# pythtb/pythtb

Hardware: AMD Instinct MI355X
Metric: k-points solved/sec (H(k)+eigh) and Berry-flux/sec, Haldane 2048^2 mesh (higher is better)
Workload: dtype f64

## Files before the change

pythtb_amd/csrc/tbk_berry.hip:

```cpp
#include <math.h>
#include <stdlib.h>
#include <string.h>
#include <algorithm>
#include "tbk_internal.h"

struct AxisSet {
    int n;
    int size[3];
    int64_t stride[3];
};

__device__ __forceinline__ int64_t axis_offset(const AxisSet& ax, int64_t s) {
    int64_t off = 0;
#pragma unroll
    for (int a = 2; a >= 0; --a) {
        if (a < ax.n) {
            const int64_t q = s / ax.size[a];
            off += (s - q * ax.size[a]) * ax.stride[a];
            s = q;
        }
    }
    return off;
}

// ... 557 lines not shown
__global__ __launch_bounds__(256) void k_flux(const FluxArgs A) {
    const int slice = blockIdx.x / A.bps;
    const int blk = blockIdx.x - slice * A.bps;
    const unsigned p = (unsigned)blk * 256u + threadIdx.x;
    const unsigned per = (unsigned)A.n0 * (unsigned)A.n1;
    double pha = 0.0;
    if (p < per) {
        const unsigned i = p / (unsigned)A.n1, j = p - i * (unsigned)A.n1;
        const int nc = A.v.ncomp;
        const int64_t plane = A.v.npts * nc;
        const int64_t base = axis_offset(A.other, slice) + (int64_t)i * A.s0 + (int64_t)j * A.s1;
        const cd* u00 = A.v.data + base * nc;
        const cd* u10 = u00 + A.s0 * nc;
        const cd* u01 = u00 + A.s1 * nc;
        const cd* u11 = u10 + A.s1 * nc;
        cd d = one_link_det<NOCC, MAXN>(u00, u10, A.occ, A.nocc, nc, plane);
        d = cmul(d, one_link_det<NOCC, MAXN>(u10, u11, A.occ, A.nocc, nc, plane));
        d = cmul(d, one_link_det<NOCC, MAXN>(u11, u01, A.occ, A.nocc, nc, plane));
        d = cmul(d, one_link_det<NOCC, MAXN>(u01, u00, A.occ, A.nocc, nc, plane));
        pha = -atan2(d.y, d.x);
        if (A.plaq) A.plaq[(int64_t)slice * per + p] = pha;
    }
    __shared__ double red[4];
    double s = pha;
#pragma unroll
    for (int off = 32; off > 0; off >>= 1) s += __shfl_xor(s, off);
    if ((threadIdx.x & 63) == 0) red[threadIdx.x >> 6] = s;
    __syncthreads();
    if (threadIdx.x == 0) A.partial[(int64_t)slice * A.bps + blk] = (red[0] + red[1]) + (red[2] + red[3]);
}

__global__ __launch_bounds__(1024) void k_flux_reduce(const double* __restrict__ partial, int bps,
                                                      double* __restrict__ totals, const DoneArgs done) {
    const double* p = partial + (int64_t)blockIdx.x * bps;
    double s0 = 0.0, s1 = 0.0, s2 = 0.0, s3 = 0.0;
    for (int i = threadIdx.x; i < bps; i += 4 * 1024) {
        const double v0 = p[i];
        const double v1 = i + 1024 < bps ? p[i + 1024] : 0.0;
        const double v2 = i + 2048 < bps ? p[i + 2048] : 0.0;
        const double v3 = i + 3072 < bps ? p[i + 3072] : 0.0;
        s0 += v0;
        s1 += v1;
        s2 += v2;
        s3 += v3;
    }
    double s = (s0 + s1) + (s2 + s3);
#pragma unroll
    for (int off = 32; off > 0; off >>= 1) s += __shfl_xor(s, off);
    __shared__ double red[16];
    if ((threadIdx.x & 63) == 0) red[threadIdx.x >> 6] = s;
    __syncthreads();
    if (threadIdx.x == 0) {
        double t = red[0];
#pragma unroll
        for (int i = 1; i < 16; ++i) t += red[i];
        red[0] = t;
    }
    if (threadIdx.x == 0) {
        totals[blockIdx.x] = red[0];
        tbk_signal_done(done);
    }
}

static int check_occ(const tbk_wfs* w, const int32_t* occ, int nocc) {
    TBK_REQUIRE(occ && nocc >= 1, TBK_EINVAL, "occ must list at least one state");
    for (int i = 0; i < nocc; ++i)
        TBK_REQUIRE(occ[i] >= 0 && occ[i] < w->view.nsta, TBK_EINVAL, "occ[%d]=%d outside 0..%d", i, occ[i],
                    w->view.nsta - 1);
    return TBK_OK;
}

static int fill_occ(const tbk_wfs* w, const int32_t* occ, int nocc, int* dst) {
    int rc = check_occ(w, occ, nocc);
    if (rc) return rc;
    TBK_REQUIRE(nocc <= TBK_MAX_NOCC, TBK_EUNSUPPORTED, "nocc=%d exceeds this build's limit of %d", nocc, TBK_MAX_NOCC);
    for (int i = 0; i < nocc; ++i) dst[i] = occ[i];
    return TBK_OK;
}

#include "tbk_berry_big.inl"
#include "tbk_berry_lanes.inl"

static int big_scratch(tbk_wfs* w, const int32_t* occ, int nocc, int ndirs, size_t extra, int** occ_dev, cd** dets,
                       void** work, size_t* work_bytes, void** extra_dev) {
    tbk_ctx* ctx = w->ctx;
    auto al = [](size_t x) { return (x + 255) & ~(size_t)255; };
    const size_t ob = al((size_t)nocc * sizeof(int));
    const size_t db = al((size_t)w->view.npts * sizeof(cd));
    const size_t per = (size_t)nocc * nocc * sizeof(cd);
    const bool in_lds = (size_t)nocc * (nocc + 1) * sizeof(cd) <= 96 * 1024;
    const size_t wb = in_lds ? 0 : al(per * (size_t)std::min<int64_t>(w->view.npts, (int64_t)ctx->cus * 4));
    void* base = nullptr;
    int rc = tbk_ctx_scratch(ctx, 256 + ob + ndirs * db + wb + al(extra), &base);
    if (rc) return rc;
// ... 20 lines not shown
        ax->stride[ax->n] = v.stride[d];
        ax->n++;
        *count *= v.mesh[d];
    }
}

template <int NOCC, int MAXN>
static void launch_flux(tbk_ctx* ctx, const FluxArgs& A, int64_t nslices) {
    hipLaunchKernelGGL((k_flux<NOCC, MAXN>), dim3((unsigned)(nslices * A.bps)), dim3(256), 0, ctx->stream, A);
}

static int chain_wave_link_dets(tbk_wfs* w, const int32_t* occ, int nocc, int dir, cd* dets_out);
#define TBK_LANES_DET_LDS_MAX ((size_t)128 * 1024)
#define TBK_LANES_FLUX_LDS_MAX ((size_t)72 * 1024)
static bool lanes_dets_applies(const WfsView& v, int nocc, size_t lds_max);
static int lanes_link_dets(tbk_wfs* w, const int32_t* occ, int nocc, int dir, cd* dets_out);
static bool chain_wave_applies(const WfsView& v, int nocc);

extern "C" int tbk_berry_flux_async(tbk_wfs* w, const int32_t* occ, int nocc, int dir0, int dir1,
                                    int want_plaq) {
    TBK_REQUIRE(w, TBK_EINVAL, "tbk_berry_flux: null wfs");
    const WfsView& v = w->view;
    TBK_REQUIRE(dir0 != dir1, TBK_EINVAL, "Need to specify two different directions for Berry flux calculation.");
    TBK_REQUIRE(dir0 >= 0 && dir1 >= 0 && dir0 < v.dim_arr && dir1 < v.dim_arr, TBK_EINVAL,
                "Direction for Berry flux calculation out of bounds.");
    FluxArgs A{};
    int det_from = 9;
    if (tbk_knobs().det_big_from >= 0) det_from = std::max(2, tbk_knobs().det_big_from);
    const bool big = nocc >= det_from;
    int rc = big ? check_occ(w, occ, nocc) : fill_occ(w, occ, nocc, A.occ);
    if (rc) return rc;
    tbk_ctx* ctx = w->ctx;
    TBK_HIP(hipSetDevice(ctx->device));
    A.v = v;
    A.nocc = nocc;
    A.n0 = v.mesh[dir0] - 1;
    A.n1 = v.mesh[dir1] - 1;
    A.s0 = v.stride[dir0];
    A.s1 = v.stride[dir1];
    int64_t nslices = 1;
    other_axes(v, dir0, dir1, &A.other, &nslices);
    const int64_t per = (int64_t)A.n0 * A.n1;
    TBK_REQUIRE(per < (int64_t)0xffffffffu, TBK_EUNSUPPORTED, "plane of %lld plaquettes is too large", (long long)per);
    const bool rows = !big && v.ncomp <= 4 && nocc <= v.ncomp;
    if (rows) {
        A.swap = A.s0 < A.s1;
        A.na = A.swap ? A.n1 : A.n0;
        A.nb = A.swap ? A.n0 : A.n1;
        A.sa = A.swap ? A.s1 : A.s0;
        A.sb = A.swap ? A.s0 : A.s1;
        A.ncolw = (A.nb + 62) / 63;
        const int64_t want = (int64_t)ctx->cus * 12;
        int64_t ti = ((int64_t)A.na * A.ncolw * nslices + want - 1) / want;
        A.ti = (int)std::max<int64_t>(4, std::min<int64_t>(24, ti));
        if (tbk_knobs().flux_ti >= 0) A.ti = std::max(1, tbk_knobs().flux_ti);
        A.bps = ((A.na + A.ti - 1) / A.ti) * A.ncolw;
    } else {
        A.bps = (int)((per + 255) / 256);
    }
    FluxSliceArgs SL{};
    const int Dm = v.dim_arr;
    const bool slices_k = rows && !want_plaq && Dm >= 3 && dir0 != Dm - 1 && dir1 != Dm - 1 && v.mesh[Dm - 1] >= 16 &&
                          tbk_knobs().flux_slices != 0;
    if (slices_k) {
        SL.nfast = v.mesh[Dm - 1];
        SL.ngrp = (SL.nfast + 63) / 64;
// ... 126 lines not shown
            }
#undef TBK_SLC
        } else if (rows) {
            const dim3 grid((unsigned)(nslices * A.bpb)), blk(256);
#define TBK_ROWS(NO, NC) hipLaunchKernelGGL((k_flux_rows<NO, NC>), grid, blk, 0, ctx->stream, A)
            switch (v.ncomp * 8 + nocc) {
                case 1 * 8 + 1: TBK_ROWS(1, 1); break;
                case 2 * 8 + 1: TBK_ROWS(1, 2); break;
                case 2 * 8 + 2: TBK_ROWS(2, 2); break;
                case 3 * 8 + 1: TBK_ROWS(1, 3); break;
                case 3 * 8 + 2: TBK_ROWS(2, 3); break;
                case 3 * 8 + 3: TBK_ROWS(3, 3); break;
                case 4 * 8 + 1: TBK_ROWS(1, 4); break;
                case 4 * 8 + 2: TBK_ROWS(2, 4); break;
                case 4 * 8 + 3: TBK_ROWS(3, 4); break;
                default: TBK_ROWS(4, 4); break;
            }
#undef TBK_ROWS
        } else {
            switch (nocc) {
                case 1: launch_flux<1, 1>(ctx, A, nslices); break;
                case 2: launch_flux<2, 1>(ctx, A, nslices); break;
                case 3: launch_flux<3, 1>(ctx, A, nslices); break;
                case 4: launch_flux<4, 1>(ctx, A, nslices); break;
                case 5: launch_flux<5, 1>(ctx, A, nslices); break;
                case 6: launch_flux<6, 1>(ctx, A, nslices); break;
                case 7: launch_flux<7, 1>(ctx, A, nslices); break;
                case 8: launch_flux<8, 1>(ctx, A, nslices); break;
                default: launch_flux<0, TBK_MAX_NOCC>(ctx, A, nslices);
            }
        }
        TBK_HIP(hipGetLastError());
    }
    if (!rows || !A.fused || slices_k) {
        ProfScope ps(ctx, "flux_reduce");
        w->flux_done = (w->flux_totals_host && !want_plaq) ? tbk_done_arm(ctx, false) : DoneArgs{nullptr, nullptr, nullptr, 0u};
        hipLaunchKernelGGL(k_flux_reduce, dim3((unsigned)nslices), dim3(1024), 0, ctx->stream,
                           (const double*)w->flux_partial_dev, (rows && !slices_k) ? A.bpb : A.bps, w->flux_totals_dev, w->flux_done);
        TBK_HIP(hipGetLastError());
    } else {
        w->flux_done = DoneArgs{nullptr, nullptr, nullptr, 0u};
    }
    return TBK_OK;
}

extern "C" int tbk_berry_flux_result(tbk_wfs* w, double* totals, double* plaq) {
    TBK_REQUIRE(w && totals, TBK_EINVAL, "tbk_berry_flux_result: null argument");
    TBK_REQUIRE(w->flux_nslices > 0, TBK_EINVAL, "tbk_berry_flux_result: no flux launch pending");
    tbk_ctx* ctx = w->ctx;
    if (plaq) {
        TBK_REQUIRE(w->flux_plaq_n > 0, TBK_EINVAL, "tbk_berry_flux_result: plaquettes were not requested");
        TBK_HIP(hipMemcpyAsync(plaq, w->flux_plaq_dev, w->flux_plaq_n * sizeof(double), hipMemcpyDeviceToHost,
                               ctx->stream));
    }
    if (w->flux_totals_host) {
        const DoneArgs done = plaq ? DoneArgs{nullptr, nullptr, nullptr, 0u} : w->flux_done;
        w->flux_done = DoneArgs{nullptr, nullptr, nullptr, 0u};
        const int rc = tbk_done_wait(ctx, done);
        if (rc) return rc;
        memcpy(totals, w->flux_totals_host, w->flux_nslices * sizeof(double));
        return TBK_OK;
    }
    return tbk_small_d2h(ctx, totals, w->flux_totals_dev, w->flux_nslices * sizeof(double));
}

extern "C" int tbk_berry_flux(tbk_wfs* w, const int32_t* occ, int nocc, int dir0, int dir1, double* totals,
                              double* plaq) {
    int rc = tbk_berry_flux_async(w, occ, nocc, dir0, dir1, plaq != nullptr);
    if (rc) return rc;
    return tbk_berry_flux_result(w, totals, plaq);
}

struct ChainArgs {
    WfsView v;
    int nocc;
    int occ[TBK_MAX_NOCC];
    int nlinks;
    int64_t sdir;
    AxisSet other;
    int64_t nstrings;
    int seg_len, nseg;
    int final_lanes;
// ... 1184 lines not shown
```

pythtb_amd/csrc/tbk_core.hip:

```cpp
#include <stdarg.h>
#include <stdio.h>
#include <stdlib.h>
#include <string.h>
#include <algorithm>
#include <array>
#include <chrono>
#include <map>
#include <new>
#include "tbk_internal.h"
#include <cmath>

static thread_local char g_err[1024] = "";

void tbk_set_error(const char* fmt, ...) {
    va_list ap;
    va_start(ap, fmt);
    vsnprintf(g_err, sizeof(g_err), fmt, ap);
    va_end(ap);
}

extern "C" const char* tbk_last_error(void) { return g_err; }

static TbkKnobs g_knobs;
static bool g_knobs_parsed = false;
// ... 18 lines not shown
    geti("TBK_QL32", k.ql32);
    geti("TBK_QLW_STREAMS", k.qlw_streams);
    geti("TBK_QLW_BISECT", k.qlw_bisect);
    geti("TBK_QLW_REPLAY_REG", k.qlw_replay_reg);
    geti("TBK_QLW_WS_MB", k.qlw_ws_mb);
    getl("TBK_QLW_CAP", k.qlw_cap);
    geti("TBK_QL16_EVONLY", k.ql16_evonly);
    geti("TBK_TW16", k.tw16);
    geti("TBK_E16", k.e16);
    geti("TBK_E16_NS_FULL", k.e16_ns_full);
    geti("TBK_E16_CELLS", k.e16_cells);
    geti("TBK_E16_EVALS", k.e16_evals);
    geti("TBK_TW16_STREAMS", k.tw16_streams);
    if (const char* e = getenv("TBK_TW16_GAPTOL")) k.tw16_gaptol = atof(e);
    geti("TBK_QL16_SPLIT", k.ql16_split);
    getl("TBK_QL16_SPLIT_MIN", k.ql16_split_min);
    getl("TBK_QL16_MIN", k.ql16_min);
    getl("TBK_FEW_MAX", k.few_max);
    geti("TBK_FEW_WARM", k.few_warm);
    geti("TBK_FEW_NT", k.few_nt);
    geti("TBK_WG_NT", k.wg_nt);
    geti("TBK_WAVE_RUN", k.wave_run);
    geti("TBK_GRID_SEG", k.grid_seg);
    geti("TBK_FUSED_ROWS", k.fused_rows);
    geti("TBK_FUSED_SUM", k.fused_sum);
    geti("TBK_FUSED_OCC", k.fused_occ);
    geti("TBK_GRID_OCC", k.grid_occ);
    geti("TBK_SMALL_KPT", k.small_kpt);
    geti("TBK_ZERO_COPY_KB", k.zero_copy_kb);
    geti("TBK_GRID_KERNEL", k.grid_kernel);
    geti("TBK_FLUX_TI", k.flux_ti);
    geti("TBK_FLUX_FUSED", k.flux_fused);
    geti("TBK_FLUX_ORDER", k.flux_order);
    geti("TBK_REG_DIRECT", k.reg_direct);
    geti("TBK_REG_CELLS", k.reg_cells);
    geti("TBK_FLUX_SLICES", k.flux_slices);
    geti("TBK_POLL_DONE", k.poll_done);
    geti("TBK_POS_TILE", k.pos_tile);
    geti("TBK_GRID_IMG", k.grid_img);
    geti("TBK_CHAIN_WAVE", k.chain_wave);
    geti("TBK_CHAIN_TILE", k.chain_tile);
    geti("TBK_CHAIN_PROD", k.chain_prod);
    geti("TBK_MESH_ROWS", k.mesh_rows);
    geti("TBK_TRIGV_FROM", k.trigv_from);
    geti("TBK_CHAIN_WS_MB", k.chain_ws_mb);
    geti("TBK_CHAIN_WAVE_FROM", k.chain_wave_from);
    geti("TBK_DET_BIG_FROM", k.det_big_from);
    geti("TBK_WILSON_BIG_FROM", k.wilson_big_from);
    geti("TBK_WILSON_REG", k.wilson_reg);
    geti("TBK_WILSON_SEG", k.wilson_seg);
    geti("TBK_WILSON_SWZ", k.wilson_swz);
    geti("TBK_WILSON_FORM", k.wilson_form);
    geti("TBK_WILSON_MFMA", k.wilson_mfma);
    getl("TBK_WILSON_BATCH_BYTES", k.wilson_batch_bytes);
    if (const char* e = getenv("TBK_WILSON_ALPHA")) {
        k.wilson_alpha = atof(e);
        k.wilson_alpha_set = true;
    }
    getl("TBK_BIG_BATCH", k.big_batch);
#ifdef TBK_REG_MULTILANE
    geti("TBK_REG_LANES", k.reg_lanes);
#endif
#ifdef TBK_DIAG
    geti("TBK_ABLATE_GRID", k.ablate_grid);
    geti("TBK_ABLATE_FLUX", k.ablate_flux);
#endif
// ... 165 lines not shown
    if (!c->done_host || tbk_knobs().poll_done == 0 || c->prof_period != 0) return d;
    c->done_seq += 1u;
    if (c->done_seq == 0u) c->done_seq = 1u;
    d.word = c->done_dev;
    d.cnt = c->done_cnt_dev;
    d.flags_src = with_flags ? c->flags_dev : nullptr;
    d.seq = c->done_seq;
    return d;
}

int tbk_done_wait(tbk_ctx* c, const DoneArgs& d) {
    if (d.word) {
        const volatile unsigned* w = c->done_host;
        const auto t0 = std::chrono::steady_clock::now();
        for (;;) {
            for (int i = 0; i < 512; ++i) {
                if ((int)(__atomic_load_n(w, __ATOMIC_ACQUIRE) - d.seq) >= 0) return TBK_OK;
                __builtin_ia32_pause();
            }
            if (std::chrono::steady_clock::now() - t0 > std::chrono::milliseconds(1)) break;
        }
    }
    TBK_HIP(hipStreamSynchronize(c->stream));
    return TBK_OK;
}

void tbk_wfs_totals_free(tbk_wfs* w) {
    if (w->flux_totals_host) hipHostFree(w->flux_totals_host);
    else if (w->flux_totals_dev) hipFree(w->flux_totals_dev);
    w->flux_totals_host = nullptr;
    w->flux_totals_dev = nullptr;
}
int tbk_wfs_totals_alloc(tbk_wfs* w, int64_t nslices) {
    tbk_wfs_totals_free(w);
    const size_t bytes = (size_t)std::max<int64_t>(nslices, 1) * sizeof(double);
    if (bytes <= 64 * 1024 && tbk_knobs().zero_copy_kb > 0) {
        void* h = nullptr;
        void* d = nullptr;
        if (hipHostMalloc(&h, bytes, hipHostMallocMapped) == hipSuccess && hipHostGetDevicePointer(&d, h, 0) == hipSuccess) {
            w->flux_totals_host = (double*)h;
            w->flux_totals_dev = (double*)d;
            return TBK_OK;
        }
        (void)hipGetLastError();
        if (h) hipHostFree(h);
    }
    TBK_HIP(hipMalloc((void**)&w->flux_totals_dev, bytes));
    return TBK_OK;
}

int tbk_ctx_scratch(tbk_ctx* c, size_t bytes, void** out) {
    if (bytes > c->scratch_bytes) {
        TBK_HIP(hipStreamSynchronize(c->stream));
        if (c->scratch) TBK_HIP(hipFree(c->scratch));
        c->scratch = nullptr;
        c->scratch_bytes = 0;
        size_t want = std::max(bytes, (size_t)1 << 20);
        hipError_t e = hipMalloc(&c->scratch, want);
        if (e != hipSuccess) {
            tbk_set_error("device scratch of %zu bytes: %s", want, hipGetErrorString(e));
            return TBK_ENOMEM;
        }
        c->scratch_bytes = want;
    }
    *out = c->scratch;
    return TBK_OK;
// ... 783 lines not shown
```

pythtb_amd/csrc/tbk_internal.h:

```cpp
#pragma once
#include <hip/hip_runtime.h>
#include <stdint.h>
#include <string>
#include <vector>
#include "../../include/tbk.h"

void tbk_set_error(const char* fmt, ...);

#define TBK_HIP(call)                                                                   \
    do {                                                                                \
        hipError_t e_ = (call);                                                         \
        if (e_ != hipSuccess) {                                                         \
            tbk_set_error("%s failed: %s (%s:%d)", #call, hipGetErrorString(e_),        \
                          __FILE__, __LINE__);                                          \
            return TBK_EHIP;                                                            \
        }                                                                               \
    } while (0)

#define TBK_REQUIRE(cond, code, ...)                                                    \
    do {                                                                                \
        if (!(cond)) {                                                                  \
            tbk_set_error(__VA_ARGS__);                                                 \
            return (code);                                                              \
        }                                                                               \
// ... 21 lines not shown
    int qlw_nt = -1;
    long long qlw_cap = -1;
    int qlw_ws_mb = -1;
    int ql16_split = 1;
    long long ql16_split_min = -1;
    int tw16_streams = -1;
    int e16 = 1;
    int tw16 = 1;
    int e16_evals = 1;
    int e16_cells = 1;
    int e16_ns_full = 0;
    double tw16_gaptol = 1e-5;
    int ql16_evonly = 1;
    long long few_max = -1;
    int few_warm = 1;
    int few_nt = -1;
    int wg_nt = 1024;
    int wave_run = -1;
    int fused_rows = -1;
    int zero_copy_kb = 1024;
    int small_kpt = -1;
    int grid_occ = -1;
    int fused_occ = -1;
    int fused_sum = 1;
    int grid_seg = -1;
    int grid_kernel = 0;
    int flux_ti = -1;
    int grid_img = 1;
    int pos_tile = 1;
    int poll_done = 1;
    int flux_slices = 1;
    int flux_fused = 0;
    int flux_order = -1;
    int trigv_from = -1;
    int chain_ws_mb = 1024;
    int mesh_rows = 1;
    int chain_prod = 1;
    int chain_tile = 1;
    int chain_wave = 1;
    int chain_wave_from = -1;
    int det_big_from = -1;
    int wilson_mfma = 1;
    int wilson_reg = 3;
    int wilson_seg = -1;
    int wilson_swz = 1;
    int wilson_form = -1;
    int wilson_big_from = -1;
    long long wilson_batch_bytes = -1;
    double wilson_alpha = 0.0;
    bool wilson_alpha_set = false;
    long long big_batch = -1;
    int reg_lanes = 0;
    int reg_cells = 1;
    int reg_direct = 1;
    int ablate_grid = 0;
    int ablate_flux = 0;
};
const TbkKnobs& tbk_knobs();

#ifdef TBK_DIAG
#define TBK_ABLATE(expr) (expr)
#else
#define TBK_ABLATE(expr) 0
#endif

struct cd {
// ... 104 lines not shown
};

int tbk_ctx_scratch(tbk_ctx* ctx, size_t bytes, void** out);
int tbk_ctx_zero_copy(tbk_ctx* ctx, size_t bytes, void** host, void** dev);
int tbk_small_d2h(tbk_ctx* ctx, void* dst, const void* src_dev, size_t bytes);
int tbk_small_result(tbk_ctx* ctx, void* dst, const void* src_dev, size_t bytes, int* flags_out);

#define TBK_PINNED_BYTES ((size_t)1 << 20)
#define TBK_FLAG_LISTED 16
struct DoneArgs {
    unsigned* word;
    unsigned* cnt;
    const int* flags_src;
    unsigned seq;
};
DoneArgs tbk_done_arm(tbk_ctx* ctx, bool with_flags);
int tbk_done_wait(tbk_ctx* ctx, const DoneArgs& d);
#ifdef __HIPCC__
__device__ inline void tbk_signal_done(const DoneArgs& d) {
    if (!d.word) return;
    __threadfence_system();
    const unsigned t = atomicAdd(d.cnt, 1u);
    if (t == gridDim.x * gridDim.y * gridDim.z - 1u) {
        __hip_atomic_store(d.cnt, 0u, __ATOMIC_RELAXED, __HIP_MEMORY_SCOPE_AGENT);
        if (d.flags_src) {
#pragma unroll
            for (int i = 0; i < 4; ++i)
                d.word[4 + i] = (unsigned)__hip_atomic_load(d.flags_src + i, __ATOMIC_RELAXED, __HIP_MEMORY_SCOPE_AGENT);
        }
        __threadfence_system();
        __hip_atomic_store(d.word, d.seq, __ATOMIC_RELEASE, __HIP_MEMORY_SCOPE_SYSTEM);
    }
}
#endif

struct ProfScope {
    tbk_ctx* ctx;
    const char* name;
    hipEvent_t t0 = nullptr, t1 = nullptr;
    ProfScope(tbk_ctx* c, const char* n);
    ~ProfScope();
};

struct ModelView {
    int dim_k;
    int nsta;
    int nspin;
    int nslot;
    const int32_t* slot_ptr;
    const int32_t* slot_ab;
    const cd* term_amp;
    const int4* term_R;
    const double4* orb;
    int pmax;
    const int32_t* cell_ptr;
    int nR;
    const int4* rvec;
    const cd* rblock;
    int nnz;
    const int4* nz;
    int pairs_hint;
};

struct tbk_model {
    tbk_ctx* ctx = nullptr;
    int dim_k = 0, norb = 0, nspin = 1, nsta = 0, nslot = 0;
// ... 14 lines not shown
    cd* data;
};
__device__ __forceinline__ cd* wf_at(const WfsView& v, int band, int64_t point) {
    return v.data + ((int64_t)band * v.npts + point) * v.ncomp;
}

#define TBK_GAP_SHARDS 64

struct tbk_wfs {
    tbk_ctx* ctx = nullptr;
    WfsView view{};
    int64_t bytes = 0;
    unsigned long long* gaps_dev = nullptr;
    int gaps_n = 0, gaps_parity = 0;
    double* gap_part_dev = nullptr;
    int64_t gap_part_cap = 0, gap_part_n = 0;
    cd* pbc_dev = nullptr;
    struct tbk_model* last_model = nullptr;
    double last_start[TBK_MAX_DIM] = {0.0, 0.0, 0.0, 0.0};
    int64_t last_off[TBK_MAX_DIM] = {0, 0, 0, 0}, last_gmesh[TBK_MAX_DIM] = {1, 1, 1, 1};
    std::vector<double> last_pbc;
    cd* tab_dev = nullptr;
    int64_t tab_cap = 0;
    std::vector<double> tab_key;
    double* flux_totals_dev = nullptr;
    double* flux_totals_host = nullptr;
    DoneArgs flux_done{nullptr, nullptr, nullptr, 0u};
    unsigned* flux_cnt_dev = nullptr;
    int64_t flux_nslices = 0, flux_nslices_cap = 0;
    double* flux_plaq_dev = nullptr;
    int64_t flux_plaq_cap = 0, flux_plaq_n = 0;
    double* flux_partial_dev = nullptr;
    int64_t flux_partial_cap = 0;
};

int tbk_mesh_evals_rows(struct tbk_model* m, const int32_t* mesh, double* e_dev, bool* done);
int tbk_wfs_totals_alloc(struct tbk_wfs* w, int64_t nslices);
void tbk_wfs_totals_free(struct tbk_wfs* w);

int tbk_eigh_dev(tbk_ctx* ctx, int n, const cd* ham_dev, int64_t nk, double* eval_dev, cd* evec_dev,
                 const char* name);
int tbk_eigh_check(tbk_ctx* ctx, int n);
int tbk_eigh_dev_checked(tbk_ctx* ctx, int n, const cd* ham_dev, int64_t nk, double* eval_dev, cd* evec_dev, const char* name);
```

pythtb_amd/csrc/tbk_solve.hip:

```cpp
#include <math.h>
#include <stdlib.h>
#include <string.h>
#include <algorithm>
#include <type_traits>
#include "tbk_internal.h"
#include <cstring>

#include "tbk_solve_dev.h"

template <int N>
struct SmallMat {
    double dg[N];
    cd up[N][N];
    cd v[N][N];
};

template <int N, int P, int Q, bool VEC>
__device__ __forceinline__ void rotate(SmallMat<N>& M) {
    const cd g = M.up[P][Q];
    const double g2 = cabs2(g);
    if (g2 > 0.0) {
        const double a = 0.5 * (M.dg[Q] - M.dg[P]), aa = fabs(a);
        const double r = sqrt(a * a + g2);
        const double inv = rsqrt(2.0 * r * (r + aa));
// ... 883 lines not shown
#pragma unroll
        for (int b = a; b < N; ++b, ++slot) {
            const cd* Cs = C + slot * npow + pmax;
            cd acc = Cs[0];
            cd zp = zl;
            if constexpr (PM >= 0) {
#pragma unroll
                for (int p = 1; p <= PM; ++p) {
                    cfma_x(acc, Cs[p], zp);
                    cfmac_x(acc, Cs[-p], zp);
                    if (p < PM) zp = cmul_x(zp, zl);
                }
            } else {
                for (int p = 1; p <= pmax; ++p) {
                    cfma_x(acc, Cs[p], zp);
                    cfmac_x(acc, Cs[-p], zp);
                    zp = cmul_x(zp, zl);
                }
            }
            if (b == a) dg[a] = acc.x;
            else up[a][b] = acc;
            if ((slot & 1) == 1) __builtin_amdgcn_sched_barrier(0);
        }
    }
}
__device__ __forceinline__ double uniform_d(const double v) {
    const I2 i = __builtin_bit_cast(I2, v);
    return __builtin_bit_cast(double, I2{__builtin_amdgcn_readfirstlane(i.lo), __builtin_amdgcn_readfirstlane(i.hi)});
}

#ifndef TBK_ROWS_OCC
#define TBK_ROWS_OCC
#endif
template <int N, int PM>
__global__ __launch_bounds__(256) TBK_ROWS_OCC void k_grid_rows(const ModelView mv, const GridArgs G) {
    extern __shared__ __align__(16) unsigned char lds_rows[];
    constexpr int NSLOT = N * (N + 1) / 2;
    const int wib = N > 2 ? __builtin_amdgcn_readfirstlane((int)(threadIdx.x >> 6)) : (int)(threadIdx.x >> 6);
    const int lane = threadIdx.x & 63;
    const int pmax = PM >= 0 ? PM : mv.pmax;
    const int npow = 2 * pmax + 1;
    const int ncell = NSLOT * npow;
    cd* C = reinterpret_cast<cd*>(lds_rows) + wib * ncell;
    cd* stage = reinterpret_cast<cd*>(lds_rows) + 4 * ncell + wib * rows_stage_slots(N);
    const int64_t tile = (int64_t)blockIdx.x * 4 + wib;
    const bool live = tile < G.ntiles;
    const int last = G.last;
    const int nlast = G.wv.mesh[last];
    const int ncol = G.img_last ? nlast - 1 : nlast;
    unsigned row = 0;
    int jc0 = 0, jc1 = 0;
    cd frow[N];
#pragma unroll
    for (int o = 0; o < N; ++o) frow[o] = cd{1.0, 0.0};
    if (live) {
        row = (unsigned)(tile / G.tpr);
        if constexpr (N > 2) row = (unsigned)__builtin_amdgcn_readfirstlane((int)row);
        const int ts = (int)(tile - (int64_t)row * G.tpr);
        jc0 = ts * G.seg;
        jc1 = min(jc0 + G.seg, G.cpr);
        cd z[4] = {cd{1.0, 0.0}, cd{1.0, 0.0}, cd{1.0, 0.0}, cd{1.0, 0.0}};
        unsigned rem = row;
#pragma unroll
        for (int d = 2; d >= 0; --d) {
            if (d < last) {
                const unsigned md = (unsigned)G.wv.mesh[d];
                const unsigned q = rem / md;
                const unsigned id = rem - q * md;
                rem = q;
// ... 1558 lines not shown
    if (key != w->tab_key) {
        std::vector<cd> st((size_t)TBK_MAX_DIM * n, cd{0.0, 0.0});
        for (int d = 0; d < D; ++d)
            for (int o = 0; o < n; ++o)
                st[d * n + o] = cd{pbc_phase[2 * (d * n + o)], pbc_phase[2 * (d * n + o) + 1]};
        TBK_HIP(hipMemcpyAsync(w->pbc_dev, st.data(), st.size() * sizeof(cd), hipMemcpyHostToDevice, ctx->stream));
        TBK_HIP(hipStreamSynchronize(ctx->stream));
        ProfScope ps(ctx, "grid_tables");
        hipLaunchKernelGGL(k_grid_tables, dim3((unsigned)((ntab + 255) / 256)), dim3(256), 0, ctx->stream, m->view, G,
                           w->tab_dev, w->tab_dev + ntab, w->tab_dev + ntab * (1 + n));
        TBK_HIP(hipGetLastError());
        w->tab_key = key;
    }
    const size_t half = (size_t)TBK_GAP_SHARDS * w->view.ncomp;
    G.gaps = w->gaps_dev + (size_t)w->gaps_parity * half;
    G.gaps_next = w->gaps_dev + (size_t)(1 - w->gaps_parity) * half;
    w->gaps_parity = 1 - w->gaps_parity;
    w->gaps_n = n - 1;
    w->gap_part_n = 0;
    G.last = D - 1;
    G.cpr = (v.mesh[D - 1] + 63) / 64;
    G.nchunks = (v.npts / v.mesh[D - 1]) * G.cpr;
    G.reg_cells = tbk_knobs().reg_cells != 0 && G.gmesh[D - 1] >= 32 ? 1 : 0;
#ifdef TBK_DIAG
    G.ablate = tbk_knobs().ablate_grid;
#endif
    if (ff) {
        const int pm = m->view.pmax;
        TBK_REQUIRE(D == 2 && (n == 2 || n == 4) && ff->nocc <= n && pm >= 0 && pm <= 2 && (n == 2 || pm == 1) &&
                        tbk_knobs().grid_kernel != 1 && v.npts < (int64_t)0x7fffffff,
                    TBK_EUNSUPPORTED, "tbk_wfs_solve_grid_flux: a %d-D array of %d states (last-axis range %d): the fused kernel "
                    "serves 2-D arrays of 2 states (range <= 2) or 4 states (range 1)", D, n, pm);
        const TbkKnobs& K = tbk_knobs();
        FusedArgs F{};
        const bool in_llc = w->bytes <= ((int64_t)256 << 20) + (1 << 20);
        F.R = K.fused_rows > 0 ? std::min(K.fused_rows, 16) : (in_llc ? 6 : 8);
        F.nrg = (v.mesh[0] + F.R - 1) / F.R;
        F.occ[0] = ff->occ[0];
        F.occ[1] = ff->occ[1];
        const int64_t want = (int64_t)ctx->cus * 32;
        const int R1 = F.R + 1, ncell = (n * (n + 1) / 2) * (2 * pm + 1), ncar = ff->nocc * n + 1;
        const size_t fixed_cd = (size_t)R1 * (ncell + n + ncar) + (size_t)64 * n;
        const int seg_cap = (int)std::max<size_t>(1, (1024 - std::min<size_t>(fixed_cd, 960)) / ((size_t)64 * (1 + n)));
        G.seg = (int)std::max<int64_t>(1, std::min<int64_t>(std::min<int64_t>(seg_cap, G.cpr), (int64_t)G.cpr * F.nrg / want));
        if (!in_llc) G.seg = 1;
        if (K.grid_seg >= 0) G.seg = std::max(1, std::min(std::min(K.grid_seg, seg_cap), G.cpr));
        G.tpr = (G.cpr + G.seg - 1) / G.seg;
        G.seg = (G.cpr + G.tpr - 1) / G.tpr;
        G.ntiles = (int64_t)F.nrg * G.tpr;
        const int nseam = G.tpr - 1;
        const int64_t seam_threads = (int64_t)(v.mesh[0] - 1) * nseam;
        const int64_t nsb = (seam_threads + 255) / 256;
        const int64_t npart = G.ntiles * std::max(n - 1, 1);
        if (w->gap_part_cap < npart) {
            TBK_HIP(hipStreamSynchronize(ctx->stream));
            if (w->gap_part_dev) TBK_HIP(hipFree(w->gap_part_dev));
            w->gap_part_dev = nullptr;
            w->gap_part_cap = 0;
            TBK_HIP(hipMalloc((void**)&w->gap_part_dev, (size_t)npart * sizeof(double)));
            w->gap_part_cap = npart;
        }
        G.gap_part = w->gap_part_dev;
        w->gap_part_n = G.ntiles;
        if (w->flux_nslices_cap < 1) {
            TBK_HIP(hipStreamSynchronize(ctx->stream));
            if (w->flux_cnt_dev) TBK_HIP(hipFree(w->flux_cnt_dev));
// ... 52 lines not shown
        else TBK_SEAMS(4, 2);
#undef TBK_SEAMS
        if (own_sum)
            hipLaunchKernelGGL(k_sum_fixed, dim3(1), dim3(1024), 0, ctx->stream, (const double*)F.partial, (int64_t)(G.ntiles + sblocks), w->flux_totals_dev);
        TBK_HIP(hipGetLastError());
        return TBK_OK;
    }
    ProfScope ps(ctx, "solve_grid");
    if (n <= 4) {
        TBK_REQUIRE(v.npts / v.mesh[D - 1] < (int64_t)0xffffffffu && G.nchunks < (int64_t)0x7fffffff * 4, TBK_EUNSUPPORTED,
                    "tbk_wfs_solve_grid: mesh too large for 32-bit row indices");
        const int64_t nrows = v.npts / v.mesh[D - 1];
        const int64_t want = (int64_t)ctx->cus * (n > 2 ? 64 : 32);
        const size_t lds_rows_need = ((size_t)4 * (n * (n + 1) / 2) * (2 * m->view.pmax + 1) + (size_t)4 * rows_stage_slots(n)) * sizeof(cd);
        const bool rows_kernel = lds_rows_need <= 48 * 1024 && tbk_knobs().grid_kernel != 1;
        G.img_last = rows_kernel && tbk_knobs().grid_img != 0 && v.mesh[D - 1] >= 2 && G.off[D - 1] == 0 && v.mesh[D - 1] == G.gmesh[D - 1] ? 1 : 0;
        if (G.img_last) {
            G.cpr = (v.mesh[D - 1] - 1 + 63) / 64;
            G.nchunks = nrows * G.cpr;
        }
        G.img_win = rows_kernel && n > 2 && !G.img_last && G.off[D - 1] + v.mesh[D - 1] == G.gmesh[D - 1] ? 1 : 0;
        G.seg = (int)std::max<int64_t>(1, std::min<int64_t>(std::min<int64_t>(8, G.cpr), G.nchunks / want));
        if (tbk_knobs().grid_seg >= 0) G.seg = std::max(1, std::min(tbk_knobs().grid_seg, G.cpr));
        G.tpr = (G.cpr + G.seg - 1) / G.seg;
        G.seg = (G.cpr + G.tpr - 1) / G.tpr;
        G.ntiles = nrows * G.tpr;
        size_t lds = lds_rows_need;
        if (lds <= 48 * 1024 && tbk_knobs().grid_kernel != 1) {
            TBK_REQUIRE(tbk_knobs().grid_occ != 1, TBK_EINVAL,
                        "TBK_GRID_OCC=1 asks for %d bytes of LDS per workgroup (limit 65536 without a function attribute): use 2..7",
                        160 * 1024 / 2 + 1024);
            if (tbk_knobs().grid_occ > 0 && tbk_knobs().grid_occ < 8)
                lds = std::max(lds, (size_t)(160 * 1024) / (size_t)(tbk_knobs().grid_occ + 1) + 1024);
            const unsigned blocks = (unsigned)((G.ntiles + 3) / 4);
            const int64_t npart = G.ntiles * std::max(n - 1, 1);
            if (w->gap_part_cap < npart) {
                TBK_HIP(hipStreamSynchronize(ctx->stream));
                if (w->gap_part_dev) TBK_HIP(hipFree(w->gap_part_dev));
                w->gap_part_dev = nullptr;
                w->gap_part_cap = 0;
                TBK_HIP(hipMalloc((void**)&w->gap_part_dev, (size_t)npart * sizeof(double)));
                w->gap_part_cap = npart;
            }
            G.gap_part = w->gap_part_dev;
            w->gap_part_n = G.ntiles;
#define TBK_ROWS(NN, PP) hipLaunchKernelGGL((k_grid_rows<NN, PP>), dim3(blocks), dim3(256), lds, ctx->stream, m->view, G)
            const int pm = m->view.pmax;
            switch (n * 8 + (pm <= 4 ? pm : 5)) {
                case 8 + 0: TBK_ROWS(1, 0); break;
                case 8 + 1: TBK_ROWS(1, 1); break;
                case 8 + 2: TBK_ROWS(1, 2); break;
                case 8 + 3: case 8 + 4: case 8 + 5: TBK_ROWS(1, -1); break;
                case 16 + 0: TBK_ROWS(2, 0); break;
                case 16 + 1: TBK_ROWS(2, 1); break;
                case 16 + 2: TBK_ROWS(2, 2); break;
                case 16 + 3: TBK_ROWS(2, 3); break;
                case 16 + 4: TBK_ROWS(2, 4); break;
                case 16 + 5: TBK_ROWS(2, -1); break;
                case 24 + 0: TBK_ROWS(3, 0); break;
                case 24 + 1: TBK_ROWS(3, 1); break;
                case 24 + 2: TBK_ROWS(3, 2); break;
                case 24 + 3: TBK_ROWS(3, 3); break;
                case 24 + 4: TBK_ROWS(3, 4); break;
                case 24 + 5: TBK_ROWS(3, -1); break;
                case 32 + 0: TBK_ROWS(4, 0); break;
                case 32 + 1: TBK_ROWS(4, 1); break;
                case 32 + 2: TBK_ROWS(4, 2); break;
                case 32 + 3: TBK_ROWS(4, 3); break;
                case 32 + 4: TBK_ROWS(4, 4); break;
                default: TBK_ROWS(4, -1); break;
            }
#undef TBK_ROWS
        } else {
            const unsigned blocks = (unsigned)((G.nchunks + 3) / 4);
            switch (n) {
                case 1: hipLaunchKernelGGL((k_grid_small<1>), dim3(blocks), dim3(256), 0, ctx->stream, m->view, G); break;
                case 2: hipLaunchKernelGGL((k_grid_small<2>), dim3(blocks), dim3(256), 0, ctx->stream, m->view, G); break;
                case 3: hipLaunchKernelGGL((k_grid_small<3>), dim3(blocks), dim3(256), 0, ctx->stream, m->view, G); break;
// ... 130 lines not shown
```

pythtb_amd/csrc/tbk_solve_dev.h:

```cpp
#ifndef TBK_SOLVE_DEV_H
#define TBK_SOLVE_DEV_H
#include <math.h>
#include <stdlib.h>
#include <string.h>
#include <algorithm>
#include <type_traits>
#include "tbk_internal.h"

#define TBK_JACOBI_MAX_SWEEPS 30

struct GridArgs {
    WfsView wv;
    double start_k[TBK_MAX_DIM];
    int gmesh[TBK_MAX_DIM];
    int64_t off[TBK_MAX_DIM];
    const cd* pbc;
    unsigned long long* gaps;
    unsigned long long* gaps_next;
    double* gap_part;
    const cd* tz[TBK_MAX_DIM];
    const cd* tf[TBK_MAX_DIM];
    int last;
    int cpr;
    int64_t nchunks;
    int wnchunk;
    int64_t wcfirst;
    int* flags;
    int img_last;
    int img_win;
    const cd* tf0;
    int seg;
    int tpr;
    int64_t ntiles;
    int reg_cells;
#ifdef TBK_DIAG
    int ablate;
#endif
};

struct ListArgs {
    const double* k;
    const cd* ham;
    double* eval;
    cd* evec;
    int* flags;
    int natural;
    DoneArgs done;
};

__device__ __forceinline__ bool tbk_before(const double o, const double mine, const int j, const int x) {
    const bool on = o != o, mn = mine != mine;
    return on ? (mn && j < x) : (mn || o < mine || (o == mine && j < x));
}

__device__ __forceinline__ cd expi2pi(const double x) {
    const double f = x - __builtin_rint(x);
    const double q = __builtin_rint(4.0 * f);
    const double h = fma(q, -0.25, f);
    const double t = h + h;
    const int m = (int)q & 3;
    const double u = t * t;
    double sp = tbk_add_vs(tbk_mul_vs(u, 0.00046153185538358102), -0.0073700215869077707);
    sp = tbk_fma_vs(sp, u, 0.082145869180001746);
    sp = tbk_fma_vs(sp, u, -0.59926452893964488);
    sp = tbk_fma_vs(sp, u, 2.5501640398733763);
    sp = tbk_fma_vs(sp, u, -5.1677127800499543);
    sp = tbk_fma_vs(sp, u, 3.1415926535897931);
// ... 222 lines not shown
```

Measured before the change: 54.01 billion.

## Defer single-slice flux reduction and piggyback it onto next grid-solve launch

Instead of launching a separate k_flux_reduce kernel after a single-slice Berry flux, the reduction is recorded as pending. It is then either run as an extra workgroup appended to the next k_grid_rows launch, or flushed when results are requested or another flux call begins. The reduction body moves into a shared templated helper that works for both 1024- and 256-thread blocks. This saves one kernel launch per iteration, but adds cross-call state that must be flushed correctly, and the done-signal arming moves to result time.

```diff
diff --git a/pythtb_amd/csrc/tbk_berry.hip b/pythtb_amd/csrc/tbk_berry.hip
--- a/pythtb_amd/csrc/tbk_berry.hip
+++ b/pythtb_amd/csrc/tbk_berry.hip
@@ -613,34 +613,25 @@
 
 __global__ __launch_bounds__(1024) void k_flux_reduce(const double* __restrict__ partial, int bps,
                                                       double* __restrict__ totals, const DoneArgs done) {
-    const double* p = partial + (int64_t)blockIdx.x * bps;
-    double s0 = 0.0, s1 = 0.0, s2 = 0.0, s3 = 0.0;
-    for (int i = threadIdx.x; i < bps; i += 4 * 1024) {
-        const double v0 = p[i];
-        const double v1 = i + 1024 < bps ? p[i + 1024] : 0.0;
-        const double v2 = i + 2048 < bps ? p[i + 2048] : 0.0;
-        const double v3 = i + 3072 < bps ? p[i + 3072] : 0.0;
-        s0 += v0;
-        s1 += v1;
-        s2 += v2;
-        s3 += v3;
-    }
-    double s = (s0 + s1) + (s2 + s3);
-#pragma unroll
-    for (int off = 32; off > 0; off >>= 1) s += __shfl_xor(s, off);
     __shared__ double red[16];
-    if ((threadIdx.x & 63) == 0) red[threadIdx.x >> 6] = s;
-    __syncthreads();
+    const double t = tbk_flux_sum_fixed<1024>(partial + (int64_t)blockIdx.x * bps, bps, red);
     if (threadIdx.x == 0) {
-        double t = red[0];
-#pragma unroll
-        for (int i = 1; i < 16; ++i) t += red[i];
-        red[0] = t;
-    }
-    if (threadIdx.x == 0) {
-        totals[blockIdx.x] = red[0];
+        totals[blockIdx.x] = t;
         tbk_signal_done(done);
     }
+}
+
+int tbk_flux_flush_pending(tbk_wfs* w, bool arm) {
+    if (w->flux_pend_n <= 0) return TBK_OK;
+    tbk_ctx* ctx = w->ctx;
+    ProfScope ps(ctx, "flux_reduce");
+    w->flux_done = (arm && w->flux_totals_host) ? tbk_done_arm(ctx, false) : DoneArgs{nullptr, nullptr, nullptr, 0u};
+    hipLaunchKernelGGL(k_flux_reduce, dim3((unsigned)w->flux_pend_nslices), dim3(1024), 0, ctx->stream,
+                       (const double*)w->flux_partial_dev, w->flux_pend_n, w->flux_totals_dev, w->flux_done);
+    w->flux_pend_n = 0;
+    w->flux_pend_nslices = 0;
+    TBK_HIP(hipGetLastError());
+    return TBK_OK;
 }
 
 static int check_occ(const tbk_wfs* w, const int32_t* occ, int nocc) {
@@ -727,6 +718,8 @@
     if (rc) return rc;
     tbk_ctx* ctx = w->ctx;
     TBK_HIP(hipSetDevice(ctx->device));
+    rc = tbk_flux_flush_pending(w, false);
+    if (rc) return rc;
     A.v = v;
     A.nocc = nocc;
     A.n0 = v.mesh[dir0] - 1;
@@ -919,7 +912,11 @@
         }
         TBK_HIP(hipGetLastError());
     }
-    if (!rows || !A.fused || slices_k) {
+    if ((!rows || !A.fused || slices_k) && nslices == 1 && !want_plaq && tbk_knobs().flux_defer != 0) {
+        w->flux_pend_n = (rows && !slices_k) ? A.bpb : A.bps;
+        w->flux_pend_nslices = 1;
+        w->flux_done = DoneArgs{nullptr, nullptr, nullptr, 0u};
+    } else if (!rows || !A.fused || slices_k) {
         ProfScope ps(ctx, "flux_reduce");
         w->flux_done = (w->flux_totals_host && !want_plaq) ? tbk_done_arm(ctx, false) : DoneArgs{nullptr, nullptr, nullptr, 0u};
         hipLaunchKernelGGL(k_flux_reduce, dim3((unsigned)nslices), dim3(1024), 0, ctx->stream,
@@ -935,6 +932,10 @@
     TBK_REQUIRE(w && totals, TBK_EINVAL, "tbk_berry_flux_result: null argument");
     TBK_REQUIRE(w->flux_nslices > 0, TBK_EINVAL, "tbk_berry_flux_result: no flux launch pending");
     tbk_ctx* ctx = w->ctx;
+    {
+        const int rc = tbk_flux_flush_pending(w, true);
+        if (rc) return rc;
+    }
     if (plaq) {
         TBK_REQUIRE(w->flux_plaq_n > 0, TBK_EINVAL, "tbk_berry_flux_result: plaquettes were not requested");
         TBK_HIP(hipMemcpyAsync(plaq, w->flux_plaq_dev, w->flux_plaq_n * sizeof(double), hipMemcpyDeviceToHost,
diff --git a/pythtb_amd/csrc/tbk_core.hip b/pythtb_amd/csrc/tbk_core.hip
--- a/pythtb_amd/csrc/tbk_core.hip
+++ b/pythtb_amd/csrc/tbk_core.hip
@@ -74,6 +74,7 @@
     geti("TBK_FLUX_TI", k.flux_ti);
     geti("TBK_FLUX_FUSED", k.flux_fused);
     geti("TBK_FLUX_ORDER", k.flux_order);
+    geti("TBK_FLUX_DEFER", k.flux_defer);
     geti("TBK_REG_DIRECT", k.reg_direct);
     geti("TBK_REG_CELLS", k.reg_cells);
     geti("TBK_FLUX_SLICES", k.flux_slices);
@@ -305,6 +306,11 @@
     w->flux_totals_dev = nullptr;
 }
 int tbk_wfs_totals_alloc(tbk_wfs* w, int64_t nslices) {
+    if (w->flux_pend_n > 0) {
+        const int rc = tbk_flux_flush_pending(w, false);
+        if (rc) return rc;
+        TBK_HIP(hipStreamSynchronize(w->ctx->stream));
+    }
     tbk_wfs_totals_free(w);
     const size_t bytes = (size_t)std::max<int64_t>(nslices, 1) * sizeof(double);
     if (bytes <= 64 * 1024 && tbk_knobs().zero_copy_kb > 0) {
diff --git a/pythtb_amd/csrc/tbk_internal.h b/pythtb_amd/csrc/tbk_internal.h
--- a/pythtb_amd/csrc/tbk_internal.h
+++ b/pythtb_amd/csrc/tbk_internal.h
@@ -77,6 +77,7 @@
     int flux_slices = 1;
     int flux_fused = 0;
     int flux_order = -1;
+    int flux_defer = 1;
     int trigv_from = -1;
     int chain_ws_mb = 1024;
     int mesh_rows = 1;
@@ -247,6 +248,35 @@
         __hip_atomic_store(d.word, d.seq, __ATOMIC_RELEASE, __HIP_MEMORY_SCOPE_SYSTEM);
     }
 }
+
+template <int NT>
+__device__ __forceinline__ double tbk_flux_sum_fixed(const double* __restrict__ p, const int n, double* red) {
+    static_assert(NT % 64 == 0 && 1024 % NT == 0, "tbk_flux_sum_fixed: whole wavefronts, whole rounds");
+#pragma unroll
+    for (int r = 0; r < 1024 / NT; ++r) {
+        const int v = r * NT + (int)threadIdx.x;
+        double s0 = 0.0, s1 = 0.0, s2 = 0.0, s3 = 0.0;
+        for (int i = v; i < n; i += 4 * 1024) {
+            const double v0 = p[i];
+            const double v1 = i + 1024 < n ? p[i + 1024] : 0.0;
+            const double v2 = i + 2048 < n ? p[i + 2048] : 0.0;
+            const double v3 = i + 3072 < n ? p[i + 3072] : 0.0;
+            s0 += v0;
+            s1 += v1;
+            s2 += v2;
+            s3 += v3;
+        }
+        double s = (s0 + s1) + (s2 + s3);
+#pragma unroll
+        for (int off = 32; off > 0; off >>= 1) s += __shfl_xor(s, off);
+        if ((threadIdx.x & 63) == 0) red[v >> 6] = s;
+    }
+    __syncthreads();
+    double t = red[0];
+#pragma unroll
+    for (int i = 1; i < 16; ++i) t += red[i];
+    return t;
+}
 #endif
 
 struct ProfScope {
@@ -327,7 +357,10 @@
     int64_t flux_plaq_cap = 0, flux_plaq_n = 0;
     double* flux_partial_dev = nullptr;
     int64_t flux_partial_cap = 0;
-};
+    int flux_pend_n = 0;
+    int64_t flux_pend_nslices = 0;
+};
+int tbk_flux_flush_pending(struct tbk_wfs* w, bool arm);
 
 int tbk_mesh_evals_rows(struct tbk_model* m, const int32_t* mesh, double* e_dev, bool* done);
 int tbk_wfs_totals_alloc(struct tbk_wfs* w, int64_t nslices);
diff --git a/pythtb_amd/csrc/tbk_solve.hip b/pythtb_amd/csrc/tbk_solve.hip
--- a/pythtb_amd/csrc/tbk_solve.hip
+++ b/pythtb_amd/csrc/tbk_solve.hip
@@ -939,9 +939,19 @@
 #ifndef TBK_ROWS_OCC
 #define TBK_ROWS_OCC
 #endif
+__device__ __forceinline__ void grid_carried_flux_sum(const double* __restrict__ partial, const int n, double* __restrict__ total,
+                                                      double* red) {
+    const double t = tbk_flux_sum_fixed<256>(partial, n, red);
+    if (threadIdx.x == 0) total[0] = t;
+}
+
 template <int N, int PM>
 __global__ __launch_bounds__(256) TBK_ROWS_OCC void k_grid_rows(const ModelView mv, const GridArgs G) {
     extern __shared__ __align__(16) unsigned char lds_rows[];
+    if (G.red_n > 0 && (int64_t)blockIdx.x * 4 >= G.ntiles) {
+        grid_carried_flux_sum(G.red_partial, G.red_n, G.red_total, reinterpret_cast<double*>(lds_rows));
+        return;
+    }
     constexpr int NSLOT = N * (N + 1) / 2;
     const int wib = N > 2 ? __builtin_amdgcn_readfirstlane((int)(threadIdx.x >> 6)) : (int)(threadIdx.x >> 6);
     const int lane = threadIdx.x & 63;
@@ -2566,6 +2576,10 @@
                     TBK_EUNSUPPORTED, "tbk_wfs_solve_grid_flux: a %d-D array of %d states (last-axis range %d): the fused kernel "
                     "serves 2-D arrays of 2 states (range <= 2) or 4 states (range 1)", D, n, pm);
         const TbkKnobs& K = tbk_knobs();
+        {
+            const int rcp = tbk_flux_flush_pending(w, false);
+            if (rcp) return rcp;
+        }
         FusedArgs F{};
         const bool in_llc = w->bytes <= ((int64_t)256 << 20) + (1 << 20);
         F.R = K.fused_rows > 0 ? std::min(K.fused_rows, 16) : (in_llc ? 6 : 8);
@@ -2684,7 +2698,7 @@
                         160 * 1024 / 2 + 1024);
             if (tbk_knobs().grid_occ > 0 && tbk_knobs().grid_occ < 8)
                 lds = std::max(lds, (size_t)(160 * 1024) / (size_t)(tbk_knobs().grid_occ + 1) + 1024);
-            const unsigned blocks = (unsigned)((G.ntiles + 3) / 4);
+            unsigned blocks = (unsigned)((G.ntiles + 3) / 4);
             const int64_t npart = G.ntiles * std::max(n - 1, 1);
             if (w->gap_part_cap < npart) {
                 TBK_HIP(hipStreamSynchronize(ctx->stream));
@@ -2696,6 +2710,15 @@
             }
             G.gap_part = w->gap_part_dev;
             w->gap_part_n = G.ntiles;
+            if (w->flux_pend_n > 0 && w->flux_pend_nslices == 1) {
+                G.red_n = w->flux_pend_n;
+                G.red_partial = w->flux_partial_dev;
+                G.red_total = w->flux_totals_dev;
+                blocks += 1u;
+                lds = std::max(lds, (size_t)16 * sizeof(double));
+                w->flux_pend_n = 0;
+                w->flux_pend_nslices = 0;
+            }
 #define TBK_ROWS(NN, PP) hipLaunchKernelGGL((k_grid_rows<NN, PP>), dim3(blocks), dim3(256), lds, ctx->stream, m->view, G)
             const int pm = m->view.pmax;
             switch (n * 8 + (pm <= 4 ? pm : 5)) {
diff --git a/pythtb_amd/csrc/tbk_solve_dev.h b/pythtb_amd/csrc/tbk_solve_dev.h
--- a/pythtb_amd/csrc/tbk_solve_dev.h
+++ b/pythtb_amd/csrc/tbk_solve_dev.h
@@ -33,6 +33,9 @@
     int tpr;
     int64_t ntiles;
     int reg_cells;
+    int red_n;
+    const double* red_partial;
+    double* red_total;
 #ifdef TBK_DIAG
     int ablate;
 #endif
```

After: 56.38 billion, median of 6. +4.4%, better.
